# CuzImSlymi/Apertis-LLM

Measured on AMD Instinct MI355X. Metric: train tokens/sec/node (seq=4096), higher is better.
Workload: dtype bf16

## Files before the change

apertis_llm_amd/csrc/moe_routing.hip:

```cpp
#include "row_common.h"

namespace {

template <int EC>
__global__ void gate_topk_fwd_k(const float *__restrict__ logits, float *__restrict__ gates,
                                int32_t *__restrict__ idx, float *__restrict__ w, int64_t S, int E_rt,
                                int K) {
  const int64_t s = (int64_t)blockIdx.x * blockDim.x + threadIdx.x;
  if (s >= S) return;
  const int E = EC > 0 ? EC : E_rt;
  gate_topk_row<EC>(logits + s * E, gates + s * E, idx + s * K, w + s * K, E_rt, K);
}

template <int EC>
__global__ void gate_topk_bwd_k(const float *__restrict__ gates, const int32_t *__restrict__ idx,
                                const float *__restrict__ dw, const float *__restrict__ dgates,
                                float *__restrict__ dlogits, int64_t S, int E_rt, int K) {
  const int64_t s = (int64_t)blockIdx.x * blockDim.x + threadIdx.x;
  if (s >= S) return;
  constexpr int CAP = EC > 0 ? EC : MAXE;
  const int E = EC > 0 ? EC : E_rt;
  float g[CAP], dg[CAP];
#pragma unroll
  for (int i = 0; i < CAP; ++i)
    if (i < E) { g[i] = gates[s * E + i]; dg[i] = dgates ? dgates[s * E + i] : 0.f; }
  if (dw) {
    float psum = 0.f, dot = 0.f;
    for (int k = 0; k < K; ++k) {
      int e = idx[s * K + k];
      float pe = 0.f;
#pragma unroll
      for (int i = 0; i < CAP; ++i)
        if (i == e) pe = g[i];
      psum += pe;
      dot += dw[s * K + k] * pe;
    }
    const float den = psum + 1e-6f;
    const float corr = dot / (den * den);
    for (int k = 0; k < K; ++k) {
      int e = idx[s * K + k];
      float dp = dw[s * K + k] / den - corr;
#pragma unroll
      for (int i = 0; i < CAP; ++i)
        if (i == e) dg[i] += dp;
    }
  }
  float inner = 0.f;
#pragma unroll
  for (int i = 0; i < CAP; ++i)
    if (i < E) inner += dg[i] * g[i];
#pragma unroll
  for (int i = 0; i < CAP; ++i)
    if (i < E) dlogits[s * E + i] = g[i] * (dg[i] - inner);
}

constexpr int PLAN_HIST_BLOCKS = 512;
struct PlanWs {
  int32_t *total, *keep, *mode, *quota, *seg_start, *bpart;
  uint32_t *thr, *smask;
  int32_t *ghist;
  int32_t *done;
  int32_t *cnt_g, *cnt_t;
  int P, NCH;
};

PlanWs carve_ws(void *ws, int64_t S, int64_t E, int64_t K) {
  PlanWs w;
  w.P = (int)(E * K);
  w.NCH = (int)ceil_div64(S, 64);
  int32_t *p = (int32_t *)ws;
  w.total = p; p += w.P;
  w.keep = p; p += w.P;
  w.mode = p; p += w.P;
  w.quota = p; p += w.P;
  w.seg_start = p; p += w.P;
  w.thr = (uint32_t *)p; p += w.P;
  w.smask = (uint32_t *)p; p += w.P;
  w.ghist = p; p += (int64_t)w.P * 256;
  w.done = p; p += 4;
  w.cnt_g = p; p += (int64_t)w.P * w.NCH;
  w.cnt_t = p; p += (int64_t)w.P * w.NCH;
  w.bpart = p;
  return w;
}

__global__ void __launch_bounds__(256)
plan_hist_k(const int32_t *__restrict__ idx, int32_t *__restrict__ bpart, int64_t SK, int E, int K) {
  __shared__ int32_t h[MAXE * MAXK];
  const int P = E * K, lane = threadIdx.x & 63;
  for (int i = threadIdx.x; i < P; i += blockDim.x) h[i] = 0;
  __syncthreads();
  for (int64_t a0 = (int64_t)blockIdx.x * blockDim.x; a0 < SK; a0 += (int64_t)gridDim.x * blockDim.x) {
    const int64_t a = a0 + threadIdx.x;
    int slot = -1;
    if (a < SK) {
      const int e = idx[a];
      if (e >= 0 && e < E) slot = e * K + (int)(a % K);
    }
    unsigned long long todo = __ballot(slot >= 0);
    while (todo) {
      const int leader = __ffsll((long long)todo) - 1;
      const int s0 = __shfl(slot, leader);
      const unsigned long long m = __ballot(slot == s0);
      if (lane == leader) atomicAdd(&h[s0], __popcll(m));
      todo &= ~m;
    }
  }
  __syncthreads();
  for (int i = threadIdx.x; i < P; i += blockDim.x) bpart[(int64_t)blockIdx.x * P + i] = h[i];
}

__global__ void plan_capacity_k(PlanWs w, const uint8_t *__restrict__ active, int64_t capacity,
                                int32_t *__restrict__ offsets, int E, int K, int nhist) {
  __shared__ int32_t s_sum[256];
  {
    const int P = E * K;
    const int g = P < 256 ? 256 / P : 1;
    for (int p0 = 0; p0 < P; p0 += 256 / g) {
      const int p = p0 + (int)threadIdx.x / g, sub = (int)threadIdx.x % g;
      int t = 0;
      if (p < P && (int)threadIdx.x / g < 256 / g)
        for (int b = sub; b < nhist; b += g) t += w.bpart[(int64_t)b * P + p];
      s_sum[threadIdx.x] = t;
      __syncthreads();
      if (p < P && sub == 0 && (int)threadIdx.x / g < 256 / g) {
        int tt = 0;
        for (int q = 0; q < g; ++q) tt += s_sum[threadIdx.x + q];
        w.total[p] = tt;
      }
      __syncthreads();
    }
  }
  const int e = threadIdx.x;
  if (e < E) {
    int64_t load = 0;
    const bool on = active ? active[e] != 0 : true;
    for (int k = 0; k < K; ++k) {
      const int p = e * K + k;
      const int tot = w.total[p];
      int64_t keep = tot;
      if (!on) keep = 0;
      else if (capacity > 0) {
        int64_t rem = capacity - load;
        keep = rem <= 0 ? 0 : (tot < rem ? tot : rem);
      }
      w.keep[p] = (int)keep;
      w.mode[p] = keep == 0 ? 0 : (keep == tot ? 1 : 2);
      w.quota[p] = (int)keep;
      w.thr[p] = 0;
      w.smask[p] = 0;
      load += keep;
    }
  }
  __syncthreads();
  if (threadIdx.x == 0) {
    int run = 0;
    for (int ee = 0; ee < E; ++ee) {
      offsets[ee] = run;
      for (int k = 0; k < K; ++k) {
        w.seg_start[ee * K + k] = run;
        run += w.keep[ee * K + k];
      }
    }
    offsets[E] = run;
  }
}

__global__ void __launch_bounds__(1024)
plan_select_k(PlanWs w, const int32_t *__restrict__ idx, const float *__restrict__ wk, int64_t S, int K) {
  const int p = blockIdx.x;
  if (w.mode[p] != 2) return;
  const int e = p / K, k = p - e * K;
  __shared__ int32_t hist[256];
  __shared__ uint32_t s_prefix, s_mask;
  __shared__ int32_t s_need;
  if (threadIdx.x == 0) { s_prefix = 0; s_mask = 0; s_need = w.keep[p]; }
  for (int shift = 24; shift >= 0; shift -= 8) {
    for (int i = threadIdx.x; i < 256; i += blockDim.x) hist[i] = 0;
    __syncthreads();
    const uint32_t prefix = s_prefix, mask = s_mask;
    for (int64_t s0 = threadIdx.x; s0 < S; s0 += (int64_t)blockDim.x * 8) {
      int32_t ei[8];
      uint32_t bi[8];
#pragma unroll
      for (int u = 0; u < 8; ++u) {
        const int64_t s = s0 + (int64_t)u * blockDim.x;
        ei[u] = s < S ? idx[s * K + k] : -1;
        bi[u] = s < S ? __float_as_uint(wk[s * K + k]) : 0u;
      }
#pragma unroll
      for (int u = 0; u < 8; ++u)
        if (ei[u] == e && (bi[u] & mask) == prefix) atomicAdd(&hist[(bi[u] >> shift) & 255], 1);
    }
    __syncthreads();
    if (threadIdx.x == 0) {
      int need = s_need, cum = 0;
      for (int b = 255; b >= 0; --b) {
        if (cum + hist[b] >= need) {
          s_need = need - cum;
          s_prefix = prefix | ((uint32_t)b << shift);
          s_mask = mask | (255u << shift);
          break;
        }
        cum += hist[b];
      }
    }
    __syncthreads();
  }
  if (threadIdx.x == 0) { w.thr[p] = s_prefix; w.quota[p] = s_need; }
}

__device__ __forceinline__ void plan_sel_pick(const PlanWs &w, int p, int lane, int shift) {
  if (w.mode[p] != 2) return;
  int32_t *h = w.ghist + p * 256;
  int c[4];
#pragma unroll
  for (int j = 0; j < 4; ++j) c[j] = __hip_atomic_load(h + 255 - 4 * lane - j, __ATOMIC_RELAXED, __HIP_MEMORY_SCOPE_AGENT);
  const int mine = (c[0] + c[1]) + (c[2] + c[3]);
  int incl = mine;
#pragma unroll
  for (int off = 1; off < 64; off <<= 1) {
    const int v = __shfl_up(incl, off);
    if (lane >= off) incl += v;
  }
  const int need = w.quota[p];
  const int before = incl - mine;
  if (before < need && incl >= need) {
    int cum = before, b = 0;
#pragma unroll
    for (int j = 0; j < 4; ++j) {
      if (cum < need && cum + c[j] >= need) { b = 255 - 4 * lane - j; break; }
      cum += c[j];
    }
    w.quota[p] = need - cum;
    w.thr[p] = w.thr[p] | ((uint32_t)b << shift);
    w.smask[p] = w.smask[p] | (255u << shift);
  }
#pragma unroll
  for (int j = 0; j < 4; ++j) h[255 - 4 * lane - j] = 0;
}

__global__ void __launch_bounds__(256)
plan_sel_hist_k(PlanWs w, const int32_t *__restrict__ idx, const float *__restrict__ wk, int64_t S, int E, int K, int shift, int digit) {
  extern __shared__ int32_t lh[];
  __shared__ int32_t s_mode[32];
  __shared__ uint32_t s_mask[32], s_thr[32];
  const int P = w.P;
  for (int i = threadIdx.x; i < P * 256; i += 256) lh[i] = 0;
  if (threadIdx.x < P) { s_mode[threadIdx.x] = w.mode[threadIdx.x]; s_mask[threadIdx.x] = w.smask[threadIdx.x]; s_thr[threadIdx.x] = w.thr[threadIdx.x]; }
  __syncthreads();
  const int64_t SK = S * K;
  for (int64_t a0 = (int64_t)blockIdx.x * 256 + threadIdx.x; a0 < SK; a0 += (int64_t)gridDim.x * 256 * 4) {
    int32_t ei[4];
    uint32_t bi[4];
#pragma unroll
    for (int u = 0; u < 4; ++u) {
      const int64_t a = a0 + (int64_t)u * gridDim.x * 256;
      ei[u] = a < SK ? idx[a] : -1;
      bi[u] = a < SK ? __float_as_uint(wk[a]) : 0u;
    }
#pragma unroll
    for (int u = 0; u < 4; ++u) {
      const int64_t a = a0 + (int64_t)u * gridDim.x * 256;
      if (ei[u] >= 0 && ei[u] < E) {
        const int p = ei[u] * K + (int)(a % K);
        if (s_mode[p] == 2 && (bi[u] & s_mask[p]) == s_thr[p]) atomicAdd(&lh[p * 256 + ((bi[u] >> shift) & 255)], 1);
      }
    }
  }
  __syncthreads();
  for (int i = threadIdx.x; i < P * 256; i += 256)
    if (lh[i]) atomicAdd(&w.ghist[i], lh[i]);
  __threadfence();
  __syncthreads();
  __shared__ int s_last;
  if (threadIdx.x == 0) s_last = atomicAdd(&w.done[digit], 1) == (int)gridDim.x - 1;
  __syncthreads();
  if (!s_last) return;
  __threadfence();
  for (int p = threadIdx.x >> 6; p < P; p += 4) plan_sel_pick(w, p, threadIdx.x & 63, shift);
}

__device__ __forceinline__ void plan_flags(const PlanWs &w, const int32_t *idx, const float *wk, int64_t s,
                                           int64_t S, int k, int E, int K, int &e, bool &fg, bool &ft) {
  e = -1; fg = false; ft = false;
  if (s < S) {
    e = idx[s * K + k];
    if (e >= 0 && e < E) {
      const int p = e * K + k;
      const int m = w.mode[p];
      if (m == 1) fg = true;
      else if (m == 2) {
        uint32_t bits = __float_as_uint(wk[s * K + k]);
        uint32_t t = w.thr[p];
        fg = bits > t;
        ft = bits == t;
      }
    } else e = -1;
  }
}

__global__ void plan_count_k(PlanWs w, const int32_t *__restrict__ idx, const float *__restrict__ wk,
                             int64_t S, int E, int K) {
  const int lane = threadIdx.x & 63;
  const int64_t chunk = (int64_t)blockIdx.x * (blockDim.x >> 6) + (threadIdx.x >> 6);
  if (chunk >= w.NCH) return;
  const int64_t s = chunk * 64 + lane;
  for (int k = 0; k < K; ++k) {
    int e; bool fg, ft;
    plan_flags(w, idx, wk, s, S, k, E, K, e, fg, ft);
    for (int ee = 0; ee < E; ++ee) {
      unsigned long long bg = __ballot(e == ee && fg);
      unsigned long long bt = __ballot(e == ee && ft);
      if (lane == 0) {
        w.cnt_g[(int64_t)(ee * K + k) * w.NCH + chunk] = __popcll(bg);
        w.cnt_t[(int64_t)(ee * K + k) * w.NCH + chunk] = __popcll(bt);
      }
    }
  }
}

__global__ void __launch_bounds__(256) plan_scan_k(PlanWs w) {
  int32_t *arr = (blockIdx.x < (unsigned)w.P ? w.cnt_g + (int64_t)blockIdx.x * w.NCH
                                              : w.cnt_t + (int64_t)(blockIdx.x - w.P) * w.NCH);
  __shared__ int32_t part[256];
  const int per = (w.NCH + 255) / 256;
  const int b0 = threadIdx.x * per, b1 = min(b0 + per, w.NCH);
  int sum = 0;
  for (int i = b0; i < b1; ++i) sum += arr[i];
  part[threadIdx.x] = sum;
  __syncthreads();
  if (threadIdx.x == 0) {
    int run = 0;
    for (int i = 0; i < 256; ++i) { int t = part[i]; part[i] = run; run += t; }
  }
  __syncthreads();
  int run = part[threadIdx.x];
  for (int i = b0; i < b1; ++i) { int t = arr[i]; arr[i] = run; run += t; }
}

__global__ void plan_assign_k(PlanWs w, const int32_t *__restrict__ idx, const float *__restrict__ wk,
                              int32_t *__restrict__ row_token, int32_t *__restrict__ row_k,
                              int32_t *__restrict__ slot_of, int64_t S, int E, int K) {
  const int lane = threadIdx.x & 63;
  const int64_t chunk = (int64_t)blockIdx.x * (blockDim.x >> 6) + (threadIdx.x >> 6);
  if (chunk >= w.NCH) return;
  const int64_t s = chunk * 64 + lane;
  const unsigned long long lt = lane == 0 ? 0ull : (~0ull >> (64 - lane));
  for (int k = 0; k < K; ++k) {
    int e; bool fg, ft;
    plan_flags(w, idx, wk, s, S, k, E, K, e, fg, ft);
    int pre_g = 0, pre_t = 0;
    for (int ee = 0; ee < E; ++ee) {
      unsigned long long bg = __ballot(e == ee && fg);
      unsigned long long bt = __ballot(e == ee && ft);
      if (e == ee) { pre_g = __popcll(bg & lt); pre_t = __popcll(bt & lt); }
    }
    if (s < S) {
      int slot = -1;
      if (e >= 0 && (fg || ft)) {
        const int p = e * K + k;
        const int gb = w.cnt_g[(int64_t)p * w.NCH + chunk] + pre_g;
        const int tb = w.cnt_t[(int64_t)p * w.NCH + chunk] + pre_t;
        const int q = w.quota[p];
        if (fg || tb < q) {
          slot = w.seg_start[p] + gb + (tb < q ? tb : q);
          row_token[slot] = (int32_t)s;
          row_k[slot] = k;
        }
      }
      slot_of[s * K + k] = slot;
    }
  }
}

__global__ void __launch_bounds__(1024)
plan_small_k(const int32_t *__restrict__ idx, const float *__restrict__ wk, const uint8_t *__restrict__ active, int64_t capacity,
             int32_t *__restrict__ offsets, int32_t *__restrict__ row_token, int32_t *__restrict__ row_k,
             int32_t *__restrict__ slot_of, int S, int E, int K) {
  plan_small_body(idx, wk, active, capacity, offsets, row_token, row_k, slot_of, S, E, K, nullptr, nullptr);
}

__device__ __forceinline__ void gauss_pair(uint64_t seed, uint64_t pair, float &n0, float &n1) {
  const uint32_t h0 = drop_hash_pair(seed, 2 * pair), h1 = drop_hash_pair(seed ^ 0x9E3779B97F4A7C15ull, 2 * pair + 1);
  const float u1 = ((float)(h0 >> 8) + 1.0f) * (1.0f / 16777216.0f);
  const float u2 = (float)(h1 >> 8) * (1.0f / 16777216.0f);
  const float r = sqrtf(-2.0f * logf(u1));
  float sn, cs;
  sincospif(2.0f * u2, &sn, &cs);
  n0 = r * cs;
  n1 = r * sn;
}
__device__ __forceinline__ float softplus_gate(float x) { return x > 20.f ? x : log1pf(expf(x)); }
template <int CAP>
__device__ __forceinline__ void row_noise(uint64_t seed, int64_t s, int E, float (&nz)[CAP]) {
  const int64_t ppr = (E + 1) / 2;
#pragma unroll
  for (int i = 0; i < CAP; i += 2) {
    if (i < E) {
      float a, b;
      gauss_pair(seed, (uint64_t)(s * ppr + (i >> 1)), a, b);
      nz[i] = a;
      if (i + 1 < CAP) nz[i + 1] = b;
    }
  }
}

template <int EC>
__global__ void __launch_bounds__(256)
gate_topk_aux_fwd_k(const float *__restrict__ logits, const float *__restrict__ w_noise, float alpha, uint64_t seed,
                    float *__restrict__ gates, int32_t *__restrict__ idx,
                    float *__restrict__ w, float *__restrict__ lse, float *__restrict__ part, int64_t S, int E_rt, int K) {
  constexpr int CAP = EC > 0 ? EC : MAXE;
  const int E = EC > 0 ? EC : E_rt;
  const int64_t s = (int64_t)blockIdx.x * blockDim.x + threadIdx.x;
  const bool live = s < S;
  float v[CAP];
  float cnt[CAP];
  float l2 = 0.f;
#pragma unroll
  for (int i = 0; i < CAP; ++i) { v[i] = 0.f; cnt[i] = 0.f; }
  if (live) {
    const float *row = logits + s * E;
    float m = -INFINITY;
#pragma unroll
    for (int i = 0; i < CAP; ++i)
      if (i < E) v[i] = row[i];
    if (w_noise) {
      float nz[CAP];
      row_noise<CAP>(seed, s, E, nz);
#pragma unroll
      for (int i = 0; i < CAP; ++i)
        if (i < E) v[i] += nz[i] * (softplus_gate(w_noise[i]) * alpha);
    }
#pragma unroll
    for (int i = 0; i < CAP; ++i)
      if (i < E) m = fmaxf(m, v[i]);
    float sum = 0.f;
#pragma unroll
    for (int i = 0; i < CAP; ++i)
      if (i < E) { v[i] = expf(v[i] - m); sum += v[i]; }
    const float l = m + logf(sum);
    lse[s] = l;
    l2 = l * l;
#pragma unroll
    for (int i = 0; i < CAP; ++i)
      if (i < E) { v[i] = v[i] / sum; gates[s * E + i] = v[i]; }
    uint64_t chosen = 0;
    float p[MAXK];
    float psum = 0.f;
#pragma unroll
    for (int k = 0; k < MAXK; ++k) {
      if (k < K) {
        float best = -1.f;
        int bi = 0;
#pragma unroll
        for (int i = 0; i < CAP; ++i)
          if (i < E && !((chosen >> i) & 1) && v[i] > best) { best = v[i]; bi = i; }
        chosen |= 1ull << bi;
        idx[s * K + k] = bi;
        p[k] = best;
        psum += best;
      }
    }
    const float den = psum + 1e-6f;
#pragma unroll
    for (int k = 0; k < MAXK; ++k)
      if (k < K) w[s * K + k] = p[k] / den;
#pragma unroll
    for (int i = 0; i < CAP; ++i)
      if (i < E) cnt[i] = (float)((chosen >> i) & 1);
  }
  __shared__ float red[4][2 * MAXE + 1];
  const int lane = threadIdx.x & 63, wv = threadIdx.x >> 6;
#pragma unroll
  for (int i = 0; i < CAP; ++i) {
    if (i < E) {
      const float a = wave_sum(v[i]), b = wave_sum(cnt[i]);
      if (lane == 0) { red[wv][i] = a; red[wv][E + i] = b; }
    }
  }
  l2 = wave_sum(l2);
  if (lane == 0) red[wv][2 * E] = l2;
  __syncthreads();
  if (threadIdx.x < 2 * E + 1)
    part[(int64_t)blockIdx.x * (2 * E + 1) + threadIdx.x] =
        (red[0][threadIdx.x] + red[1][threadIdx.x]) + (red[2][threadIdx.x] + red[3][threadIdx.x]);
}

__global__ void __launch_bounds__(1024)
gate_aux_fold_k(const float *__restrict__ part, float *__restrict__ stats, int64_t nblk, int64_t S, int E, float lb_coef,
                float rz_coef) {
  __shared__ float tot[2 * MAXE + 1];
  const int lane = threadIdx.x & 63, wv = threadIdx.x >> 6;
  const int cols = 2 * E + 1;
  for (int cc = wv; cc < cols; cc += 16) {
    float a = 0.f;
    for (int64_t b = lane; b < nblk; b += 64) a += part[b * cols + cc];
    a = wave_sum(a);
    if (lane == 0) tot[cc] = a;
  }
  __syncthreads();
  if (threadIdx.x == 0) {
    float lb = 0.f;
    for (int e = 0; e < E; ++e) lb += (tot[E + e] / (float)S) * (tot[e] / (float)S);
    stats[0] = lb_coef * (float)E * lb;
    stats[1] = rz_coef * tot[2 * E] / (float)S;
  }
  if (threadIdx.x < E) stats[2 + threadIdx.x] = tot[E + threadIdx.x] / (float)S;
}

template <int EC>
__global__ void __launch_bounds__(256)
gate_topk_aux_bwd_k(const float *__restrict__ gates, const int32_t *__restrict__ idx,
                    const float *__restrict__ dw, const float *__restrict__ lse,
                    const float *__restrict__ stats, const float *__restrict__ dlb,
                    const float *__restrict__ drz, float lb_coef, float rz_coef,
                    float *__restrict__ dlogits, float *__restrict__ npart, uint64_t seed, int64_t S, int E_rt, int K) {
  const int64_t s = (int64_t)blockIdx.x * blockDim.x + threadIdx.x;
  constexpr int CAP = EC > 0 ? EC : MAXE;
  const int E = EC > 0 ? EC : E_rt;
  float dsc[CAP];
#pragma unroll
  for (int i = 0; i < CAP; ++i) dsc[i] = 0.f;
  if (s < S) {
  const float glb = dlb ? dlb[0] * lb_coef * (float)E / (float)S : 0.f;
  const float grz = drz ? drz[0] * rz_coef * 2.f * lse[s] / (float)S : 0.f;
  float g[CAP], dg[CAP];
#pragma unroll
  for (int i = 0; i < CAP; ++i)
    if (i < E) { g[i] = gates[s * E + i]; dg[i] = glb * stats[2 + i]; }
  if (dw) {
    float psum = 0.f, dot = 0.f;
    for (int k = 0; k < K; ++k) {
      int e = idx[s * K + k];
      float pe = 0.f;
#pragma unroll
      for (int i = 0; i < CAP; ++i)
        if (i == e) pe = g[i];
      psum += pe;
      dot += dw[s * K + k] * pe;
    }
    const float den = psum + 1e-6f;
    const float corr = dot / (den * den);
    for (int k = 0; k < K; ++k) {
      int e = idx[s * K + k];
      float dp = dw[s * K + k] / den - corr;
#pragma unroll
      for (int i = 0; i < CAP; ++i)
        if (i == e) dg[i] += dp;
    }
  }
  float inner = 0.f;
#pragma unroll
  for (int i = 0; i < CAP; ++i)
    if (i < E) inner += dg[i] * g[i];
  float nz[CAP];
  if (npart) row_noise<CAP>(seed, s, E, nz);
#pragma unroll
  for (int i = 0; i < CAP; ++i)
    if (i < E) {
      const float dl = g[i] * (dg[i] - inner) + grz * g[i];
      dlogits[s * E + i] = dl;
      if (npart) dsc[i] = dl * nz[i];
    }
  }
  if (npart) {
    __shared__ float red[4][MAXE];
    const int lane = threadIdx.x & 63, wv = threadIdx.x >> 6;
#pragma unroll
    for (int i = 0; i < CAP; ++i)
      if (i < E) {
        const float a = wave_sum(dsc[i]);
        if (lane == 0) red[wv][i] = a;
      }
    __syncthreads();
    if (threadIdx.x < E)
      npart[(int64_t)blockIdx.x * E + threadIdx.x] =
          (red[0][threadIdx.x] + red[1][threadIdx.x]) + (red[2][threadIdx.x] + red[3][threadIdx.x]);
  }
}

__global__ void __launch_bounds__(1024)
gate_noise_fold_k(const float *__restrict__ npart, const float *__restrict__ w_noise, float alpha, float *__restrict__ dw_noise,
                  int64_t nblk, int E) {
  const int lane = threadIdx.x & 63, wv = threadIdx.x >> 6;
  for (int e = wv; e < E; e += 16) {
    float a = 0.f;
    for (int64_t b = lane; b < nblk; b += 64) a += npart[b * E + e];
    a = wave_sum(a);
    if (lane == 0) {
      const float x = w_noise[e];
      dw_noise[e] = a * alpha * (x > 20.f ? 1.f : 1.f / (1.f + expf(-x)));
    }
  }
}

}

extern "C" int apertis_moe_gate_topk_fwd(const float *logits, float *gates, int32_t *idx, float *w,
                                         int64_t S, int64_t E, int64_t K, void *stream) {
  if (!logits || !gates || !idx || !w || S < 0) return APERTIS_ERR_ARG;
  if (E < 1 || E > MAXE || K < 1 || K > MAXK || K > E) return APERTIS_ERR_UNSUPPORTED;
  if (S == 0) return APERTIS_OK;
  hipStream_t st = (hipStream_t)stream;
  dim3 grid((unsigned)ceil_div64(S, 256)), block(256);
#define GO(EC) hipLaunchKernelGGL(gate_topk_fwd_k<EC>, grid, block, 0, st, logits, gates, idx, w, S, (int)E, (int)K)
  if (E == 4) GO(4); else if (E == 8) GO(8); else if (E == 16) GO(16); else GO(0);
#undef GO
  return apertis_check_launch();
}

extern "C" int apertis_moe_gate_topk_bwd(const float *gates, const int32_t *idx, const float *dw,
                                         const float *dgates, float *dlogits, int64_t S, int64_t E,
                                         int64_t K, void *stream) {
  if (!gates || !idx || !dlogits || S < 0) return APERTIS_ERR_ARG;
  if (E < 1 || E > MAXE || K < 1 || K > MAXK || K > E) return APERTIS_ERR_UNSUPPORTED;
  if (S == 0) return APERTIS_OK;
  hipStream_t st = (hipStream_t)stream;
  dim3 grid((unsigned)ceil_div64(S, 256)), block(256);
#define GO(EC) hipLaunchKernelGGL(gate_topk_bwd_k<EC>, grid, block, 0, st, gates, idx, dw, dgates, dlogits, S, (int)E, (int)K)
  if (E == 4) GO(4); else if (E == 8) GO(8); else if (E == 16) GO(16); else GO(0);
#undef GO
  return apertis_check_launch();
}

extern "C" int64_t apertis_moe_plan_workspace_bytes(int64_t S, int64_t E, int64_t K) {
  int64_t P = E * K, NCH = ceil_div64(S > 0 ? S : 1, 64);
  return (7 * P + 256 * P + 4 + 2 * P * NCH + PLAN_HIST_BLOCKS * P) * 4 + 64;
}

extern "C" int apertis_moe_plan(const int32_t *idx, const float *w, const uint8_t *active,
                                int64_t capacity, int32_t *expert_offsets, int32_t *row_token,
                                int32_t *row_k, int32_t *slot_of, void *ws, int64_t S, int64_t E,
                                int64_t K, void *stream) {
  if (!idx || !w || !expert_offsets || !row_token || !row_k || !slot_of || !ws || S < 0) return APERTIS_ERR_ARG;
  if (E < 1 || E > MAXE || K < 1 || K > MAXK) return APERTIS_ERR_UNSUPPORTED;
  if (S * K > 0x7fffffffLL) return APERTIS_ERR_UNSUPPORTED;
  hipStream_t st = (hipStream_t)stream;
  if (S > 0 && S <= 64 && E * K <= 16) {
    hipLaunchKernelGGL(plan_small_k, dim3(1), dim3(64 * (unsigned)(E * K)), 0, st, idx, w, active, capacity, expert_offsets,
                       row_token, row_k, slot_of, (int)S, (int)E, (int)K);
    return apertis_check_launch();
  }
  PlanWs pw = carve_ws(ws, S > 0 ? S : 1, E, K);
  int nhist = 0;
  if (S > 0) {
    nhist = (int)std::min<int64_t>(ceil_div64(S * K, 1024), PLAN_HIST_BLOCKS);
    hipLaunchKernelGGL(plan_hist_k, dim3((unsigned)nhist), dim3(256), 0, st, idx, pw.bpart, S * K, (int)E, (int)K);
  }
  hipLaunchKernelGGL(plan_capacity_k, dim3(1), dim3(256), 0, st, pw, active, capacity, expert_offsets, (int)E, (int)K, nhist);
  if (S > 0) {
    if (capacity > 0) {
      if (pw.P <= 32) {
        hipMemsetAsync(pw.ghist, 0, sizeof(int32_t) * (pw.P * 256 + 4), st);
        const unsigned nbh = (unsigned)std::min<int64_t>(ceil_div64(S * K, 1024), 512);
        for (int shift = 24; shift >= 0; shift -= 8)
          hipLaunchKernelGGL(plan_sel_hist_k, dim3(nbh), dim3(256), (size_t)pw.P * 256 * sizeof(int32_t), st, pw, idx, w, S,
                             (int)E, (int)K, shift, 3 - shift / 8);
      } else {
        hipLaunchKernelGGL(plan_select_k, dim3(pw.P), dim3(1024), 0, st, pw, idx, w, S, (int)K);
      }
    }
    dim3 cgrid((unsigned)ceil_div64(pw.NCH, 4)), cblock(256);
    hipLaunchKernelGGL(plan_count_k, cgrid, cblock, 0, st, pw, idx, w, S, (int)E, (int)K);
    hipLaunchKernelGGL(plan_scan_k, dim3(2 * pw.P), dim3(256), 0, st, pw);
    hipLaunchKernelGGL(plan_assign_k, cgrid, cblock, 0, st, pw, idx, w, row_token, row_k, slot_of, S, (int)E, (int)K);
  }
  return apertis_check_launch();
}

extern "C" int64_t apertis_moe_gate_aux_blocks(int64_t S) { return ceil_div64(S > 0 ? S : 1, 256); }

extern "C" int apertis_moe_gate_topk_noisy_aux_fwd(const float *logits, const float *w_noise, float alpha, uint64_t seed,
                                                   float *gates, int32_t *idx, float *w, float *lse, float *part, float *stats,
                                                   int64_t S, int64_t E, int64_t K, float lb_coef, float rz_coef, void *stream) {
  if (!logits || !gates || !idx || !w || !lse || !part || !stats || S <= 0) return APERTIS_ERR_ARG;
  if (E < 1 || E > MAXE || K < 1 || K > MAXK || K > E) return APERTIS_ERR_UNSUPPORTED;
  hipStream_t st = (hipStream_t)stream;
  const int64_t nblk = apertis_moe_gate_aux_blocks(S);
  dim3 grid((unsigned)nblk), block(256);
#define GO(EC) hipLaunchKernelGGL(gate_topk_aux_fwd_k<EC>, grid, block, 0, st, logits, w_noise, alpha, seed, gates, idx, w, lse, part, S, (int)E, (int)K)
  if (E == 4) GO(4); else if (E == 8) GO(8); else if (E == 16) GO(16); else GO(0);
#undef GO
  hipLaunchKernelGGL(gate_aux_fold_k, dim3(1), dim3(1024), 0, st, part, stats, nblk, S, (int)E, lb_coef, rz_coef);
  return apertis_check_launch();
}

extern "C" int apertis_moe_gate_topk_aux_fwd(const float *logits, float *gates, int32_t *idx, float *w, float *lse,
                                             float *part, float *stats, int64_t S, int64_t E, int64_t K, float lb_coef,
                                             float rz_coef, void *stream) {
  return apertis_moe_gate_topk_noisy_aux_fwd(logits, nullptr, 0.f, 0, gates, idx, w, lse, part, stats, S, E, K, lb_coef, rz_coef,
                                             stream);
}

extern "C" int apertis_moe_gate_topk_noisy_aux_bwd(const float *gates, const int32_t *idx, const float *dw, const float *lse,
                                                   const float *stats, const float *dlb, const float *drz, float lb_coef,
                                                   float rz_coef, const float *w_noise, float alpha, uint64_t seed,
                                                   float *dlogits, float *npart, float *dw_noise, int64_t S, int64_t E,
                                                   int64_t K, void *stream) {
  if (!gates || !idx || !lse || !stats || !dlogits || S < 0 || (w_noise && (!npart || !dw_noise))) return APERTIS_ERR_ARG;
  if (!w_noise) npart = nullptr;
  if (E < 1 || E > MAXE || K < 1 || K > MAXK || K > E) return APERTIS_ERR_UNSUPPORTED;
  if (S == 0) return APERTIS_OK;
  hipStream_t st = (hipStream_t)stream;
  dim3 grid((unsigned)ceil_div64(S, 256)), block(256);
#define GO(EC) hipLaunchKernelGGL(gate_topk_aux_bwd_k<EC>, grid, block, 0, st, gates, idx, dw, lse, stats, dlb, drz, lb_coef, rz_coef, dlogits, npart, seed, S, (int)E, (int)K)
  if (E == 4) GO(4); else if (E == 8) GO(8); else if (E == 16) GO(16); else GO(0);
#undef GO
  if (npart) hipLaunchKernelGGL(gate_noise_fold_k, dim3(1), dim3(1024), 0, st, npart, w_noise, alpha, dw_noise, (int64_t)grid.x, (int)E);
  return apertis_check_launch();
}

extern "C" int apertis_moe_gate_topk_aux_bwd(const float *gates, const int32_t *idx, const float *dw, const float *lse,
                                             const float *stats, const float *dlb, const float *drz, float lb_coef,
                                             float rz_coef, float *dlogits, int64_t S, int64_t E, int64_t K, void *stream) {
  return apertis_moe_gate_topk_noisy_aux_bwd(gates, idx, dw, lse, stats, dlb, drz, lb_coef, rz_coef, nullptr, 0.f, 0, dlogits,
                                             nullptr, nullptr, S, E, K, stream);
}
```

Measured before the change: 404,900.

## Compact capacity-overflow candidates before radix select in MoE plan

Adds an emit kernel that compacts the gate weights of only the partially-kept (expert, k) slots into per-block candidate buckets. The per-slot radix select then runs over these compacted candidates, held in LDS when they fit, instead of rescanning all S*K idx/weight pairs four times. This replaces the multi-launch global-histogram path and the full-scan select, and adds wave-aggregated histogram atomics. The cost is an extra kernel, a larger workspace, and a large dynamic LDS allocation per select block.

```diff
diff --git a/apertis_llm_amd/csrc/moe_routing.hip b/apertis_llm_amd/csrc/moe_routing.hip
--- a/apertis_llm_amd/csrc/moe_routing.hip
+++ b/apertis_llm_amd/csrc/moe_routing.hip
@@ -55,19 +55,23 @@
 }
 
 constexpr int PLAN_HIST_BLOCKS = 512;
+constexpr int PLAN_EMIT_PAIRS = 1024;
+constexpr int PLAN_SEL_LDS_N = 38912;
 struct PlanWs {
   int32_t *total, *keep, *mode, *quota, *seg_start, *bpart;
-  uint32_t *thr, *smask;
-  int32_t *ghist;
-  int32_t *done;
+  uint32_t *thr;
   int32_t *cnt_g, *cnt_t;
-  int P, NCH;
+  int32_t *ccount;
+  uint32_t *cand;
+  int P, NCH, NB, STRIDE;
 };
 
 PlanWs carve_ws(void *ws, int64_t S, int64_t E, int64_t K) {
   PlanWs w;
   w.P = (int)(E * K);
   w.NCH = (int)ceil_div64(S, 64);
+  w.NB = (int)ceil_div64(S * K, PLAN_EMIT_PAIRS);
+  w.STRIDE = (int)ceil_div64(PLAN_EMIT_PAIRS, K);
   int32_t *p = (int32_t *)ws;
   w.total = p; p += w.P;
   w.keep = p; p += w.P;
@@ -75,12 +79,11 @@
   w.quota = p; p += w.P;
   w.seg_start = p; p += w.P;
   w.thr = (uint32_t *)p; p += w.P;
-  w.smask = (uint32_t *)p; p += w.P;
-  w.ghist = p; p += (int64_t)w.P * 256;
-  w.done = p; p += 4;
   w.cnt_g = p; p += (int64_t)w.P * w.NCH;
   w.cnt_t = p; p += (int64_t)w.P * w.NCH;
-  w.bpart = p;
+  w.bpart = p; p += (int64_t)PLAN_HIST_BLOCKS * w.P;
+  w.ccount = p; p += E * w.NB;
+  w.cand = (uint32_t *)p;
   return w;
 }
 
@@ -148,7 +151,6 @@
       w.mode[p] = keep == 0 ? 0 : (keep == tot ? 1 : 2);
       w.quota[p] = (int)keep;
       w.thr[p] = 0;
-      w.smask[p] = 0;
       load += keep;
     }
   }
@@ -166,119 +168,179 @@
   }
 }
 
+__global__ void __launch_bounds__(256)
+plan_emit_k(PlanWs w, const int32_t *__restrict__ idx, const float *__restrict__ wk, int64_t SK, int E, int K) {
+  __shared__ int32_t s_k[MAXE], s_c[MAXE];
+  const int lane = threadIdx.x & 63;
+  if (threadIdx.x < E) { s_k[threadIdx.x] = -1; s_c[threadIdx.x] = 0; }
+  __syncthreads();
+  for (int p = threadIdx.x; p < w.P; p += 256)
+    if (w.mode[p] == 2) s_k[p / K] = p % K;
+  __syncthreads();
+  const int64_t a0 = (int64_t)blockIdx.x * PLAN_EMIT_PAIRS + threadIdx.x;
+  int32_t ei[4];
+  uint32_t bi[4];
+#pragma unroll
+  for (int u = 0; u < 4; ++u) {
+    const int64_t a = a0 + u * 256;
+    ei[u] = a < SK ? idx[a] : -1;
+    bi[u] = a < SK ? __float_as_uint(wk[a]) : 0u;
+  }
+  const unsigned long long lt = lane == 0 ? 0ull : (~0ull >> (64 - lane));
+#pragma unroll
+  for (int u = 0; u < 4; ++u) {
+    int e = -1;
+    if (ei[u] >= 0 && ei[u] < E && s_k[ei[u]] == (int)((a0 + u * 256) % K)) e = ei[u];
+    unsigned long long todo = __ballot(e >= 0);
+    while (todo) {
+      const int leader = __ffsll((long long)todo) - 1;
+      const int e0 = __builtin_amdgcn_readlane(e, leader);
+      const unsigned long long m = __ballot(e == e0);
+      int base = 0;
+      if (lane == leader) base = atomicAdd(&s_c[e0], __popcll(m));
+      base = __builtin_amdgcn_readlane(base, leader);
+      const int pos = base + __popcll(m & lt);
+      if (e == e0 && pos < w.STRIDE) w.cand[((int64_t)e0 * w.NB + blockIdx.x) * w.STRIDE + pos] = bi[u];
+      todo &= ~m;
+    }
+  }
+  __syncthreads();
+  if (threadIdx.x < E) w.ccount[(int64_t)threadIdx.x * w.NB + blockIdx.x] = s_c[threadIdx.x];
+}
+
+template <typename F>
+__device__ __forceinline__ void plan_each_candidate(const uint32_t *__restrict__ seg, const int32_t *__restrict__ cnt, int nb,
+                                                    int stride, int32_t *s_off, int32_t *s_wsum, F f) {
+  constexpr int U = 8;
+  const int lane = threadIdx.x & 63, wave = threadIdx.x >> 6;
+  int base = 0;
+  for (int b0 = 0; b0 < nb; b0 += 1024) {
+    const int nbc = min(1024, nb - b0);
+    int incl = (int)threadIdx.x < nbc ? min(cnt[b0 + threadIdx.x], stride) : 0;
+#pragma unroll
+    for (int off = 1; off < 64; off <<= 1) {
+      const int v = __shfl_up(incl, off);
+      if (lane >= off) incl += v;
+    }
+    __syncthreads();
+    if (lane == 63) s_wsum[wave] = incl;
+    __syncthreads();
+    int pre = 0, tot = 0;
+#pragma unroll
+    for (int i = 0; i < 16; ++i) {
+      const int v = s_wsum[i];
+      pre += i < wave ? v : 0;
+      tot += v;
+    }
+    s_off[threadIdx.x + 1] = pre + incl;
+    if (threadIdx.x == 0) s_off[0] = 0;
+    __syncthreads();
+    for (int j = wave; j < nbc; j += 16 * U) {
+      int o[U], c[U];
+      uint32_t v[U][2];
+#pragma unroll
+      for (int u = 0; u < U; ++u) {
+        const int jj = min(j + 16 * u, nbc - 1);
+        o[u] = s_off[jj];
+        c[u] = j + 16 * u < nbc ? s_off[jj + 1] - o[u] : 0;
+        const uint32_t *row = seg + (int64_t)(b0 + jj) * stride;
+        v[u][0] = lane < c[u] ? row[lane] : 0u;
+        v[u][1] = 64 + lane < c[u] ? row[64 + lane] : 0u;
+      }
+#pragma unroll
+      for (int u = 0; u < U; ++u) {
+        f(v[u][0], lane < c[u], base + o[u] + lane);
+        f(v[u][1], 64 + lane < c[u], base + o[u] + 64 + lane);
+        for (int i = 128 + lane; i - lane < c[u]; i += 64)
+          f(i < c[u] ? seg[(int64_t)(b0 + j + 16 * u) * stride + i] : 0u, i < c[u], base + o[u] + i);
+      }
+    }
+    base += tot;
+  }
+}
+
 __global__ void __launch_bounds__(1024)
-plan_select_k(PlanWs w, const int32_t *__restrict__ idx, const float *__restrict__ wk, int64_t S, int K) {
+plan_select_k(PlanWs w, int K) {
   const int p = blockIdx.x;
+  const int n = w.total[p], keep = w.keep[p];
   if (w.mode[p] != 2) return;
-  const int e = p / K, k = p - e * K;
-  __shared__ int32_t hist[256];
-  __shared__ uint32_t s_prefix, s_mask;
+  extern __shared__ uint32_t s_data[];
+  __shared__ int32_t hist[256], s_off[1025], s_wsum[16];
+  __shared__ uint32_t s_prefix;
   __shared__ int32_t s_need;
-  if (threadIdx.x == 0) { s_prefix = 0; s_mask = 0; s_need = w.keep[p]; }
+  const int e = p / K, lane = threadIdx.x & 63;
+  const bool in_lds = n <= PLAN_SEL_LDS_N;
+  const uint32_t *seg = w.cand + (int64_t)e * w.NB * w.STRIDE;
+  const int32_t *cnt = w.ccount + (int64_t)e * w.NB;
+  if (threadIdx.x == 0) { s_prefix = 0; s_need = keep; }
+  if (in_lds)
+    plan_each_candidate(seg, cnt, w.NB, w.STRIDE, s_off, s_wsum, [&](uint32_t bits, bool valid, int i) {
+      if (valid && i < PLAN_SEL_LDS_N) s_data[i] = bits;
+    });
+  uint32_t mask = 0;
   for (int shift = 24; shift >= 0; shift -= 8) {
     for (int i = threadIdx.x; i < 256; i += blockDim.x) hist[i] = 0;
     __syncthreads();
-    const uint32_t prefix = s_prefix, mask = s_mask;
-    for (int64_t s0 = threadIdx.x; s0 < S; s0 += (int64_t)blockDim.x * 8) {
-      int32_t ei[8];
-      uint32_t bi[8];
-#pragma unroll
-      for (int u = 0; u < 8; ++u) {
-        const int64_t s = s0 + (int64_t)u * blockDim.x;
-        ei[u] = s < S ? idx[s * K + k] : -1;
-        bi[u] = s < S ? __float_as_uint(wk[s * K + k]) : 0u;
-      }
-#pragma unroll
-      for (int u = 0; u < 8; ++u)
-        if (ei[u] == e && (bi[u] & mask) == prefix) atomicAdd(&hist[(bi[u] >> shift) & 255], 1);
-    }
+    const uint32_t prefix = s_prefix;
+    const int need = s_need;
+    int pend_d = 0, pend_c = 0;
+    auto add = [&](uint32_t bits, bool valid, int) {
+      const bool m = valid && (bits & mask) == prefix;
+      const unsigned long long act = __ballot(m);
+      if (!act) return;
+      const int d = (int)((bits >> shift) & 255u);
+      const int d0 = __builtin_amdgcn_readlane(d, __ffsll((long long)act) - 1);
+      if (__ballot(m && d == d0) == act) {
+        if (d0 != pend_d) {
+          if (pend_c && lane == 0) atomicAdd(&hist[pend_d], pend_c);
+          pend_d = d0;
+          pend_c = 0;
+        }
+        pend_c += __popcll(act);
+      } else if (m) {
+        atomicAdd(&hist[d], 1);
+      }
+    };
+    if (in_lds) {
+      for (int i0 = threadIdx.x; i0 - (int)threadIdx.x < n; i0 += 8 * 1024) {
+        uint32_t v[8];
+#pragma unroll
+        for (int u = 0; u < 8; ++u) v[u] = i0 + u * 1024 < n ? s_data[i0 + u * 1024] : 0u;
+#pragma unroll
+        for (int u = 0; u < 8; ++u) add(v[u], i0 + u * 1024 < n, 0);
+      }
+    } else {
+      plan_each_candidate(seg, cnt, w.NB, w.STRIDE, s_off, s_wsum, add);
+    }
+    if (pend_c && lane == 0) atomicAdd(&hist[pend_d], pend_c);
     __syncthreads();
-    if (threadIdx.x == 0) {
-      int need = s_need, cum = 0;
-      for (int b = 255; b >= 0; --b) {
-        if (cum + hist[b] >= need) {
-          s_need = need - cum;
-          s_prefix = prefix | ((uint32_t)b << shift);
-          s_mask = mask | (255u << shift);
-          break;
+    if (threadIdx.x < 64) {
+      int c[4];
+#pragma unroll
+      for (int j = 0; j < 4; ++j) c[j] = hist[255 - 4 * lane - j];
+      const int mine = (c[0] + c[1]) + (c[2] + c[3]);
+      int incl = mine;
+#pragma unroll
+      for (int off = 1; off < 64; off <<= 1) {
+        const int v = __shfl_up(incl, off);
+        if (lane >= off) incl += v;
+      }
+      const int before = incl - mine;
+      if (before < need && incl >= need) {
+        int cum = before, b = 0;
+#pragma unroll
+        for (int j = 0; j < 4; ++j) {
+          if (cum + c[j] >= need) { b = 255 - 4 * lane - j; break; }
+          cum += c[j];
         }
-        cum += hist[b];
-      }
-    }
+        s_need = need - cum;
+        s_prefix = prefix | ((uint32_t)b << shift);
+      }
+    }
+    mask |= 255u << shift;
     __syncthreads();
   }
   if (threadIdx.x == 0) { w.thr[p] = s_prefix; w.quota[p] = s_need; }
-}
-
-__device__ __forceinline__ void plan_sel_pick(const PlanWs &w, int p, int lane, int shift) {
-  if (w.mode[p] != 2) return;
-  int32_t *h = w.ghist + p * 256;
-  int c[4];
-#pragma unroll
-  for (int j = 0; j < 4; ++j) c[j] = __hip_atomic_load(h + 255 - 4 * lane - j, __ATOMIC_RELAXED, __HIP_MEMORY_SCOPE_AGENT);
-  const int mine = (c[0] + c[1]) + (c[2] + c[3]);
-  int incl = mine;
-#pragma unroll
-  for (int off = 1; off < 64; off <<= 1) {
-    const int v = __shfl_up(incl, off);
-    if (lane >= off) incl += v;
-  }
-  const int need = w.quota[p];
-  const int before = incl - mine;
-  if (before < need && incl >= need) {
-    int cum = before, b = 0;
-#pragma unroll
-    for (int j = 0; j < 4; ++j) {
-      if (cum < need && cum + c[j] >= need) { b = 255 - 4 * lane - j; break; }
-      cum += c[j];
-    }
-    w.quota[p] = need - cum;
-    w.thr[p] = w.thr[p] | ((uint32_t)b << shift);
-    w.smask[p] = w.smask[p] | (255u << shift);
-  }
-#pragma unroll
-  for (int j = 0; j < 4; ++j) h[255 - 4 * lane - j] = 0;
-}
-
-__global__ void __launch_bounds__(256)
-plan_sel_hist_k(PlanWs w, const int32_t *__restrict__ idx, const float *__restrict__ wk, int64_t S, int E, int K, int shift, int digit) {
-  extern __shared__ int32_t lh[];
-  __shared__ int32_t s_mode[32];
-  __shared__ uint32_t s_mask[32], s_thr[32];
-  const int P = w.P;
-  for (int i = threadIdx.x; i < P * 256; i += 256) lh[i] = 0;
-  if (threadIdx.x < P) { s_mode[threadIdx.x] = w.mode[threadIdx.x]; s_mask[threadIdx.x] = w.smask[threadIdx.x]; s_thr[threadIdx.x] = w.thr[threadIdx.x]; }
-  __syncthreads();
-  const int64_t SK = S * K;
-  for (int64_t a0 = (int64_t)blockIdx.x * 256 + threadIdx.x; a0 < SK; a0 += (int64_t)gridDim.x * 256 * 4) {
-    int32_t ei[4];
-    uint32_t bi[4];
-#pragma unroll
-    for (int u = 0; u < 4; ++u) {
-      const int64_t a = a0 + (int64_t)u * gridDim.x * 256;
-      ei[u] = a < SK ? idx[a] : -1;
-      bi[u] = a < SK ? __float_as_uint(wk[a]) : 0u;
-    }
-#pragma unroll
-    for (int u = 0; u < 4; ++u) {
-      const int64_t a = a0 + (int64_t)u * gridDim.x * 256;
-      if (ei[u] >= 0 && ei[u] < E) {
-        const int p = ei[u] * K + (int)(a % K);
-        if (s_mode[p] == 2 && (bi[u] & s_mask[p]) == s_thr[p]) atomicAdd(&lh[p * 256 + ((bi[u] >> shift) & 255)], 1);
-      }
-    }
-  }
-  __syncthreads();
-  for (int i = threadIdx.x; i < P * 256; i += 256)
-    if (lh[i]) atomicAdd(&w.ghist[i], lh[i]);
-  __threadfence();
-  __syncthreads();
-  __shared__ int s_last;
-  if (threadIdx.x == 0) s_last = atomicAdd(&w.done[digit], 1) == (int)gridDim.x - 1;
-  __syncthreads();
-  if (!s_last) return;
-  __threadfence();
-  for (int p = threadIdx.x >> 6; p < P; p += 4) plan_sel_pick(w, p, threadIdx.x & 63, shift);
 }
 
 __device__ __forceinline__ void plan_flags(const PlanWs &w, const int32_t *idx, const float *wk, int64_t s,
@@ -626,8 +688,10 @@
 }
 
 extern "C" int64_t apertis_moe_plan_workspace_bytes(int64_t S, int64_t E, int64_t K) {
-  int64_t P = E * K, NCH = ceil_div64(S > 0 ? S : 1, 64);
-  return (7 * P + 256 * P + 4 + 2 * P * NCH + PLAN_HIST_BLOCKS * P) * 4 + 64;
+  if (E < 1 || K < 1) return 64;
+  const int64_t Sp = S > 0 ? S : 1, P = E * K, NCH = ceil_div64(Sp, 64);
+  const int64_t NB = ceil_div64(Sp * K, PLAN_EMIT_PAIRS), STRIDE = ceil_div64(PLAN_EMIT_PAIRS, K);
+  return (6 * P + 2 * P * NCH + PLAN_HIST_BLOCKS * P + E * NB * (1 + STRIDE)) * 4 + 64;
 }
 
 extern "C" int apertis_moe_plan(const int32_t *idx, const float *w, const uint8_t *active,
@@ -652,15 +716,8 @@
   hipLaunchKernelGGL(plan_capacity_k, dim3(1), dim3(256), 0, st, pw, active, capacity, expert_offsets, (int)E, (int)K, nhist);
   if (S > 0) {
     if (capacity > 0) {
-      if (pw.P <= 32) {
-        hipMemsetAsync(pw.ghist, 0, sizeof(int32_t) * (pw.P * 256 + 4), st);
-        const unsigned nbh = (unsigned)std::min<int64_t>(ceil_div64(S * K, 1024), 512);
-        for (int shift = 24; shift >= 0; shift -= 8)
-          hipLaunchKernelGGL(plan_sel_hist_k, dim3(nbh), dim3(256), (size_t)pw.P * 256 * sizeof(int32_t), st, pw, idx, w, S,
-                             (int)E, (int)K, shift, 3 - shift / 8);
-      } else {
-        hipLaunchKernelGGL(plan_select_k, dim3(pw.P), dim3(1024), 0, st, pw, idx, w, S, (int)K);
-      }
+      hipLaunchKernelGGL(plan_emit_k, dim3((unsigned)pw.NB), dim3(256), 0, st, pw, idx, w, S * K, (int)E, (int)K);
+      launch_lds(plan_select_k, dim3(pw.P), dim3(1024), (size_t)PLAN_SEL_LDS_N * sizeof(uint32_t), st, pw, (int)K);
     }
     dim3 cgrid((unsigned)ceil_div64(pw.NCH, 4)), cblock(256);
     hipLaunchKernelGGL(plan_count_k, cgrid, cblock, 0, st, pw, idx, w, S, (int)E, (int)K);
```

After: 410,000, median of 6. 1.01x the previous value.

## Replace last-block atomic pick with separate pick kernel in MoE radix select

Applied to the files above, without the earlier changes.

The radix-select histogram kernel no longer uses a done-counter with threadfences so that the last block performs the digit pick. Instead, a separate small pick kernel runs after each digit pass, one block per slot. The ghist memset is folded into the capacity kernel, and the histogram grid is capped at 256 blocks instead of 512. This removes grid-wide fences and atomics and one memset launch, at the cost of four extra small kernel launches per plan call.

```diff
diff --git a/apertis_llm_amd/csrc/moe_routing.hip b/apertis_llm_amd/csrc/moe_routing.hip
--- a/apertis_llm_amd/csrc/moe_routing.hip
+++ b/apertis_llm_amd/csrc/moe_routing.hip
@@ -55,11 +55,13 @@
 }
 
 constexpr int PLAN_HIST_BLOCKS = 512;
+#ifndef PLAN_SEL_BLOCKS
+#define PLAN_SEL_BLOCKS 256
+#endif
 struct PlanWs {
   int32_t *total, *keep, *mode, *quota, *seg_start, *bpart;
   uint32_t *thr, *smask;
   int32_t *ghist;
-  int32_t *done;
   int32_t *cnt_g, *cnt_t;
   int P, NCH;
 };
@@ -77,7 +79,6 @@
   w.thr = (uint32_t *)p; p += w.P;
   w.smask = (uint32_t *)p; p += w.P;
   w.ghist = p; p += (int64_t)w.P * 256;
-  w.done = p; p += 4;
   w.cnt_g = p; p += (int64_t)w.P * w.NCH;
   w.cnt_t = p; p += (int64_t)w.P * w.NCH;
   w.bpart = p;
@@ -111,7 +112,9 @@
 }
 
 __global__ void plan_capacity_k(PlanWs w, const uint8_t *__restrict__ active, int64_t capacity,
-                                int32_t *__restrict__ offsets, int E, int K, int nhist) {
+                                int32_t *__restrict__ offsets, int E, int K, int nhist, int zero_ghist) {
+  if (zero_ghist)
+    for (int i = threadIdx.x; i < w.P * 256; i += blockDim.x) w.ghist[i] = 0;
   __shared__ int32_t s_sum[256];
   {
     const int P = E * K;
@@ -215,7 +218,7 @@
   int32_t *h = w.ghist + p * 256;
   int c[4];
 #pragma unroll
-  for (int j = 0; j < 4; ++j) c[j] = __hip_atomic_load(h + 255 - 4 * lane - j, __ATOMIC_RELAXED, __HIP_MEMORY_SCOPE_AGENT);
+  for (int j = 0; j < 4; ++j) c[j] = h[255 - 4 * lane - j];
   const int mine = (c[0] + c[1]) + (c[2] + c[3]);
   int incl = mine;
 #pragma unroll
@@ -241,7 +244,7 @@
 }
 
 __global__ void __launch_bounds__(256)
-plan_sel_hist_k(PlanWs w, const int32_t *__restrict__ idx, const float *__restrict__ wk, int64_t S, int E, int K, int shift, int digit) {
+plan_sel_hist_k(PlanWs w, const int32_t *__restrict__ idx, const float *__restrict__ wk, int64_t S, int E, int K, int shift) {
   extern __shared__ int32_t lh[];
   __shared__ int32_t s_mode[32];
   __shared__ uint32_t s_mask[32], s_thr[32];
@@ -271,14 +274,10 @@
   __syncthreads();
   for (int i = threadIdx.x; i < P * 256; i += 256)
     if (lh[i]) atomicAdd(&w.ghist[i], lh[i]);
-  __threadfence();
-  __syncthreads();
-  __shared__ int s_last;
-  if (threadIdx.x == 0) s_last = atomicAdd(&w.done[digit], 1) == (int)gridDim.x - 1;
-  __syncthreads();
-  if (!s_last) return;
-  __threadfence();
-  for (int p = threadIdx.x >> 6; p < P; p += 4) plan_sel_pick(w, p, threadIdx.x & 63, shift);
+}
+
+__global__ void __launch_bounds__(64) plan_sel_pick_k(PlanWs w, int shift) {
+  plan_sel_pick(w, blockIdx.x, threadIdx.x, shift);
 }
 
 __device__ __forceinline__ void plan_flags(const PlanWs &w, const int32_t *idx, const float *wk, int64_t s,
@@ -627,7 +626,7 @@
 
 extern "C" int64_t apertis_moe_plan_workspace_bytes(int64_t S, int64_t E, int64_t K) {
   int64_t P = E * K, NCH = ceil_div64(S > 0 ? S : 1, 64);
-  return (7 * P + 256 * P + 4 + 2 * P * NCH + PLAN_HIST_BLOCKS * P) * 4 + 64;
+  return (7 * P + 256 * P + 2 * P * NCH + PLAN_HIST_BLOCKS * P) * 4 + 64;
 }
 
 extern "C" int apertis_moe_plan(const int32_t *idx, const float *w, const uint8_t *active,
@@ -649,15 +648,18 @@
     nhist = (int)std::min<int64_t>(ceil_div64(S * K, 1024), PLAN_HIST_BLOCKS);
     hipLaunchKernelGGL(plan_hist_k, dim3((unsigned)nhist), dim3(256), 0, st, idx, pw.bpart, S * K, (int)E, (int)K);
   }
-  hipLaunchKernelGGL(plan_capacity_k, dim3(1), dim3(256), 0, st, pw, active, capacity, expert_offsets, (int)E, (int)K, nhist);
+  const bool radix = S > 0 && capacity > 0 && pw.P <= 32;
+  hipLaunchKernelGGL(plan_capacity_k, dim3(1), dim3(256), 0, st, pw, active, capacity, expert_offsets, (int)E, (int)K, nhist,
+                     (int)radix);
   if (S > 0) {
     if (capacity > 0) {
-      if (pw.P <= 32) {
-        hipMemsetAsync(pw.ghist, 0, sizeof(int32_t) * (pw.P * 256 + 4), st);
-        const unsigned nbh = (unsigned)std::min<int64_t>(ceil_div64(S * K, 1024), 512);
-        for (int shift = 24; shift >= 0; shift -= 8)
+      if (radix) {
+        const unsigned nbh = (unsigned)std::min<int64_t>(ceil_div64(S * K, 1024), PLAN_SEL_BLOCKS);
+        for (int shift = 24; shift >= 0; shift -= 8) {
           hipLaunchKernelGGL(plan_sel_hist_k, dim3(nbh), dim3(256), (size_t)pw.P * 256 * sizeof(int32_t), st, pw, idx, w, S,
-                             (int)E, (int)K, shift, 3 - shift / 8);
+                             (int)E, (int)K, shift);
+          hipLaunchKernelGGL(plan_sel_pick_k, dim3(pw.P), dim3(64), 0, st, pw, shift);
+        }
       } else {
         hipLaunchKernelGGL(plan_select_k, dim3(pw.P), dim3(1024), 0, st, pw, idx, w, S, (int)K);
       }
```

New measurement: 397,600 before, 401,400 after, median of 6. About the same (+1.0%).
